# Teque5/caf_cookoff

Measured on NVIDIA B200. Metric: CAF cells/s (400x8192 fp64 surface + peak), higher is better.
Workload: dtype f64

## Files before the change

### caf_cookoff_b200/csrc/caf_kernels.cuh

```cuda
#pragma once
#include <cstdint>
#include <type_traits>
#include "fft16.cuh"

namespace caf {

constexpr int kThreads = 512;
constexpr int kL0 = 4096;
constexpr int kM = 8192;

enum Mode : int {
    kSurface = 0,
    kSpectrumHalf = 1,
    kSpectrumFull = 2,
    kXcorFull = 3,
    kXcorHalf = 4
};

struct PeakOut {
    double value;
    double freq_hz;
    unsigned long long doppler_idx;
    unsigned long long delay_idx;
};

template <typename T>
struct RowArgs {
    const cx<T>* in;
    const cx<T>* in2;
    cx<T>* hperm;
    const double* freqs;
    void* out;
    T* row_peak_val;
    unsigned long long* row_peak_idx;
    PeakOut* peak;
    unsigned long long* peak_words;
    unsigned long long row_offset;
    unsigned int* peak_seq;
    unsigned int seq_val;
    unsigned int* done_counter;
    unsigned int done_last;
    const cx<T>* tw1;
    const cx<T>* tw2;
    const cx<T>* g;
    double dt;
    int L;
    int D;
    int P;
    cx<T>* hshare;
    unsigned int* hflag;
    unsigned int epoch;
    int hprod1;
    const uint4* pull_src;
    uint4* pull_dst;
    unsigned int pull_n16;
    unsigned int* pull_counter;
    unsigned int pull_target;
    unsigned int flags;
    long long* trace;
};

template <typename T> struct Fab;
template <> struct Fab<double> {
    using E = double;
    static constexpr int kRegion = 280;
    static constexpr int kPlane = 16 * kRegion;
    static constexpr int kPipe = 2 * kPlane;
    static __device__ __forceinline__ void st(E* p, int i, double2 v) { p[i] = v.x; p[kPlane + i] = v.y; }
    static __device__ __forceinline__ double2 ld(const E* p, int i) { return make_double2(p[i], p[kPlane + i]); }
};
template <> struct Fab<float> {
    using E = float2;
    static constexpr int kRegion = 256;
    static constexpr int kPipe = 16 * kRegion;
    static __device__ __forceinline__ void st(E* p, int i, float2 v) { p[i] = v; }
    static __device__ __forceinline__ float2 ld(const E* p, int i) { return p[i]; }
};

template <typename T>
struct SmemLayout {
    static constexpr size_t kS = sizeof(typename Fab<T>::E) * 2 * Fab<T>::kPipe;
    static constexpr size_t kPtab = sizeof(cx<T>) * 2 * 2 * 48;
    static constexpr size_t kRed = 16 * 8 + 16 * 8;
    static constexpr size_t kCand = 2 * 256 * (8 + 4);
    static constexpr size_t kMisc = 64;
    static constexpr size_t kNeedle = sizeof(T) * 2 * kL0;
    static constexpr size_t offPtab = kS, offRed = offPtab + kPtab, offCand = offRed + kRed, offMisc = offCand + kCand,
                            offNeedle = offMisc + kMisc;
    static constexpr size_t kTotalNoNeedle = offNeedle;
    static constexpr size_t kTotal = offNeedle + kNeedle;
};

template <typename T>
struct Ctx {
    static constexpr bool kPadded = std::is_same<T, double>::value;
    typename Fab<T>::E* Sr;
    cx<T>* ptab;
    uint32_t tm_A;
    uint32_t tm_B;
    uint32_t tm_g;
    int w, lane, r, h, t;
    int wb;
    int hs[2];
    int hr;
    long long* tr;

    __device__ __forceinline__ void init(unsigned char* smem_raw, int tid) {
        const int hw_warp = tid >> 5;
        lane = tid & 31; r = tid >> 8;
        h = (lane & 7) | ((lane >> 1) & 8);
        const int sub = (lane >> 3) & 1;
        w = 2 * (hw_warp & 7) + sub;
        t = 16 * w + h;
        wb = Fab<T>::kRegion * w;
        hs[0] = h ^ (sub << 3); hs[1] = hs[0] ^ 8;
        hr = h ^ (((sub ^ h) & 1) << 3);
        Sr = reinterpret_cast<typename Fab<T>::E*>(smem_raw) + r * Fab<T>::kPipe;
        ptab = nullptr; tm_A = tm_B = tm_g = 0; tr = nullptr;
    }
    __device__ __forceinline__ int ix_block(int k) const {
        if constexpr (kPadded) return k * Fab<T>::kRegion + (t ^ ((t & 16) >> 1));
        else return k * 256 + 16 * w + hs[k & 1];
    }
    __device__ __forceinline__ int ix_own(int i) const {
        if constexpr (kPadded) return wb + 16 * i + (h ^ ((i & 1) << 3));
        else return wb + 16 * i + hs[i & 1];
    }
    __device__ __forceinline__ int ix_tw(int k) const {
        if constexpr (kPadded) return wb + 17 * k + h;
        else return wb + 16 * k + (hs[k & 1] ^ k);
    }
    __device__ __forceinline__ int ix_tr(int m) const {
        if constexpr (kPadded) return wb + 17 * h + m;
        else return wb + 16 * h + (m ^ hr);
    }
};

#ifdef CAF_TRACE
#define CAF_TR(c_, slot_) do { if ((c_).tr && (c_).lane == 0) (c_).tr[slot_] = clock64(); } while (0)
#else
#define CAF_TR(c_, slot_) do { } while (0)
#endif

__device__ __forceinline__ void tmem_ld_x16(uint32_t taddr, uint32_t (&r)[16]) {
    asm volatile("tcgen05.ld.sync.aligned.32x32b.x16.b32 {%0,%1,%2,%3,%4,%5,%6,%7,%8,%9,%10,%11,%12,%13,%14,%15}, [%16];\n"
                 : "=r"(r[0]), "=r"(r[1]), "=r"(r[2]), "=r"(r[3]), "=r"(r[4]), "=r"(r[5]), "=r"(r[6]), "=r"(r[7]),
                   "=r"(r[8]), "=r"(r[9]), "=r"(r[10]), "=r"(r[11]), "=r"(r[12]), "=r"(r[13]), "=r"(r[14]), "=r"(r[15])
                 : "r"(taddr) : "memory");
}
__device__ __forceinline__ void tmem_st_x16(uint32_t taddr, const uint32_t (&r)[16]) {
    asm volatile("tcgen05.st.sync.aligned.32x32b.x16.b32 [%0], {%1,%2,%3,%4,%5,%6,%7,%8,%9,%10,%11,%12,%13,%14,%15,%16};\n"
                 :: "r"(taddr), "r"(r[0]), "r"(r[1]), "r"(r[2]), "r"(r[3]), "r"(r[4]), "r"(r[5]), "r"(r[6]), "r"(r[7]),
                    "r"(r[8]), "r"(r[9]), "r"(r[10]), "r"(r[11]), "r"(r[12]), "r"(r[13]), "r"(r[14]), "r"(r[15]) : "memory");
}
__device__ __forceinline__ void tmem_ld_x8(uint32_t taddr, uint32_t (&r)[8]) {
    asm volatile("tcgen05.ld.sync.aligned.32x32b.x8.b32 {%0,%1,%2,%3,%4,%5,%6,%7}, [%8];\n"
                 : "=r"(r[0]), "=r"(r[1]), "=r"(r[2]), "=r"(r[3]), "=r"(r[4]), "=r"(r[5]), "=r"(r[6]), "=r"(r[7])
                 : "r"(taddr) : "memory");
}
__device__ __forceinline__ void tmem_st_x8(uint32_t taddr, const uint32_t (&r)[8]) {
    asm volatile("tcgen05.st.sync.aligned.32x32b.x8.b32 [%0], {%1,%2,%3,%4,%5,%6,%7,%8};\n"
                 :: "r"(taddr), "r"(r[0]), "r"(r[1]), "r"(r[2]), "r"(r[3]), "r"(r[4]), "r"(r[5]), "r"(r[6]), "r"(r[7]) : "memory");
}
__device__ __forceinline__ void tmem_wait_ld() { asm volatile("tcgen05.wait::ld.sync.aligned;\n" ::: "memory"); }
__device__ __forceinline__ void tmem_wait_st() { asm volatile("tcgen05.wait::st.sync.aligned;\n" ::: "memory"); }

__device__ __forceinline__ void tmem_ld_x4(uint32_t taddr, uint32_t (&r)[4]) {
    asm volatile("tcgen05.ld.sync.aligned.32x32b.x4.b32 {%0,%1,%2,%3}, [%4];\n"
                 : "=r"(r[0]), "=r"(r[1]), "=r"(r[2]), "=r"(r[3]) : "r"(taddr) : "memory");
}
__device__ __forceinline__ void tmem_st_x4(uint32_t taddr, const uint32_t (&r)[4]) {
    asm volatile("tcgen05.st.sync.aligned.32x32b.x4.b32 [%0], {%1,%2,%3,%4};\n"
                 :: "r"(taddr), "r"(r[0]), "r"(r[1]), "r"(r[2]), "r"(r[3]) : "memory");
}
__device__ __forceinline__ void tmem_ld_x2(uint32_t taddr, uint32_t (&r)[2]) {
    asm volatile("tcgen05.ld.sync.aligned.32x32b.x2.b32 {%0,%1}, [%2];\n" : "=r"(r[0]), "=r"(r[1]) : "r"(taddr) : "memory");
}
__device__ __forceinline__ void tmem_st_x2(uint32_t taddr, const uint32_t (&r)[2]) {
    asm volatile("tcgen05.st.sync.aligned.32x32b.x2.b32 [%0], {%1,%2};\n" :: "r"(taddr), "r"(r[0]), "r"(r[1]) : "memory");
}

template <typename T> struct TmemGeom;
template <> struct TmemGeom<double> { static constexpr int kColsPerC = 4, kAlloc = 512; };
template <> struct TmemGeom<float>  { static constexpr int kColsPerC = 2, kAlloc = 256; };

struct Raw4d { uint32_t r[16]; };
struct Raw4f { uint32_t r[8]; };
template <typename T> struct raw4_of;
template <> struct raw4_of<double> { using type = Raw4d; };
template <> struct raw4_of<float>  { using type = Raw4f; };
__device__ __forceinline__ void tmem_ld4_issue(uint32_t taddr, Raw4d& q) { tmem_ld_x16(taddr, q.r); }
__device__ __forceinline__ void tmem_ld4_issue(uint32_t taddr, Raw4f& q) { tmem_ld_x8(taddr, q.r); }
__device__ __forceinline__ void tmem_unpack4(const Raw4d& q, double2 (&o)[4]) {
#pragma unroll
    for (int i = 0; i < 4; ++i) {
        o[i].x = __hiloint2double((int)q.r[4 * i + 1], (int)q.r[4 * i]);
        o[i].y = __hiloint2double((int)q.r[4 * i + 3], (int)q.r[4 * i + 2]);
    }
}
__device__ __forceinline__ void tmem_unpack4(const Raw4f& q, float2 (&o)[4]) {
#pragma unroll
    for (int i = 0; i < 4; ++i) { o[i].x = __uint_as_float(q.r[2 * i]); o[i].y = __uint_as_float(q.r[2 * i + 1]); }
}
__device__ __forceinline__ void tmem_st4(uint32_t taddr, const double2 (&v)[4]) {
    uint32_t r[16];
#pragma unroll
    for (int i = 0; i < 4; ++i) {
        r[4 * i] = (uint32_t)__double2loint(v[i].x); r[4 * i + 1] = (uint32_t)__double2hiint(v[i].x);
        r[4 * i + 2] = (uint32_t)__double2loint(v[i].y); r[4 * i + 3] = (uint32_t)__double2hiint(v[i].y);
    }
    tmem_st_x16(taddr, r);
}
__device__ __forceinline__ void tmem_st4(uint32_t taddr, const float2 (&v)[4]) {
    uint32_t r[8];
#pragma unroll
    for (int i = 0; i < 4; ++i) { r[2 * i] = __float_as_uint(v[i].x); r[2 * i + 1] = __float_as_uint(v[i].y); }
    tmem_st_x8(taddr, r);
}

__device__ __forceinline__ double2 tmem_ld1(uint32_t taddr, double) {
    uint32_t r[4];
    tmem_ld_x4(taddr, r);
    tmem_wait_ld();
    return make_double2(__hiloint2double((int)r[1], (int)r[0]), __hiloint2double((int)r[3], (int)r[2]));
}
__device__ __forceinline__ float2 tmem_ld1(uint32_t taddr, float) {
    uint32_t r[2];
    tmem_ld_x2(taddr, r);
    tmem_wait_ld();
    return make_float2(__uint_as_float(r[0]), __uint_as_float(r[1]));
}
__device__ __forceinline__ void tmem_st1(uint32_t taddr, double2 v) {
    uint32_t r[4] = {(uint32_t)__double2loint(v.x), (uint32_t)__double2hiint(v.x), (uint32_t)__double2loint(v.y), (uint32_t)__double2hiint(v.y)};
    tmem_st_x4(taddr, r);
}
__device__ __forceinline__ void tmem_st1(uint32_t taddr, float2 v) {
    uint32_t r[2] = {__float_as_uint(v.x), __float_as_uint(v.y)};
    tmem_st_x2(taddr, r);
}

template <typename T>
__device__ __forceinline__ cx<T> ldg(const cx<T>* p) { return __ldg(p); }

__device__ __forceinline__ double2 unit_phasor(double n, double phi, double exact_sub) {
    double hi = n * phi;
    double lo = fma(n, phi, -hi);
    double fr = (hi - rint(hi)) + lo - exact_sub;
    fr -= rint(fr);
    double s, c;
    sincospi(2.0 * fr, &s, &c);
    return make_double2(c, s);
}

__device__ __forceinline__ void bar_group(int r) { asm volatile("bar.sync %0, 256;\n" :: "r"(r + 1) : "memory"); }

__device__ __forceinline__ void mbar_init(uint64_t* mb, int count) {
    asm volatile("mbarrier.init.shared::cta.b64 [%0], %1;\n" :: "r"((uint32_t)__cvta_generic_to_shared(mb)), "r"(count) : "memory");
}
__device__ __forceinline__ void mbar_arrive(uint64_t* mb) {
    asm volatile("{\n.reg .b64 st;\nmbarrier.arrive.shared::cta.b64 st, [%0];\n}\n"
                 :: "r"((uint32_t)__cvta_generic_to_shared(mb)) : "memory");
}
__device__ __forceinline__ void mbar_wait(uint64_t* mb, int parity) {
    const uint32_t addr = (uint32_t)__cvta_generic_to_shared(mb);
    asm volatile("{\n.reg .pred p;\nWAIT_%=:\nmbarrier.try_wait.parity.shared::cta.b64 p, [%0], %1;\n@p bra DONE_%=;\nbra WAIT_%=;\nDONE_%=:\n}\n"
                 :: "r"(addr), "r"(parity) : "memory");
}

template <typename T>
__device__ __forceinline__ void tmem_store_power_table(uint32_t taddr, cx<T> w) {
    constexpr int kC = TmemGeom<T>::kColsPerC;
    const cx<T> w2 = csq(w), w4 = csq(w2);
    cx<T> q[4];
    q[0] = mk<T>((T)1, (T)0); q[1] = w4; q[2] = csq(w4); q[3] = cmul(q[2], w4);
    tmem_st4(taddr, q);
    q[0] = w; q[1] = cmul(q[0], w4); q[2] = cmul(q[1], w4); q[3] = cmul(q[2], w4);
    tmem_st4(taddr + 4 * kC, q);
    q[0] = w2; q[1] = cmul(q[0], w4); q[2] = cmul(q[1], w4); q[3] = cmul(q[2], w4);
    tmem_st4(taddr + 8 * kC, q);
    q[0] = cmul(w2, w); q[1] = cmul(q[0], w4); q[2] = cmul(q[1], w4); q[3] = cmul(q[2], w4);
    tmem_st4(taddr + 12 * kC, q);
}

template <typename T, bool INV, int MODE, bool Q0_ONE>
__device__ __forceinline__ void fft16_in_tmem(cx<T> (&v)[16], uint32_t taddr) {
    constexpr int kC = TmemGeom<T>::kColsPerC;
    typename raw4_of<T>::type r0, r1, r2, r3;
    cx<T> q[4];
    tmem_ld4_issue(taddr, r0);
    tmem_wait_ld();
    tmem_ld4_issue(taddr + 4 * kC, r1);
    tmem_unpack4(r0, q);
    radix4_in<T, INV, MODE, Q0_ONE>(v[0], v[4], v[8], v[12], q[0], q[1], q[2], q[3]);
    tmem_wait_ld();
    tmem_ld4_issue(taddr + 8 * kC, r2);
    tmem_unpack4(r1, q);
    radix4_in<T, INV, MODE, false>(v[1], v[5], v[9], v[13], q[0], q[1], q[2], q[3]);
    tmem_wait_ld();
    tmem_ld4_issue(taddr + 12 * kC, r3);
    tmem_unpack4(r2, q);
    radix4_in<T, INV, MODE, false>(v[2], v[6], v[10], v[14], q[0], q[1], q[2], q[3]);
    tmem_wait_ld();
    tmem_unpack4(r3, q);
    radix4_in<T, INV, MODE, false>(v[3], v[7], v[11], v[15], q[0], q[1], q[2], q[3]);
    fft16_stage_b<T, INV>(v);
}

template <typename T, int MODE>
__device__ __forceinline__ void mul_table_tmem(cx<T> (&v)[16], uint32_t taddr) {
    constexpr int kC = TmemGeom<T>::kColsPerC;
    typename raw4_of<T>::type r0, r1, r2, r3;
    cx<T> q[4];
    tmem_ld4_issue(taddr, r0);
    tmem_ld4_issue(taddr + 4 * kC, r1);
    tmem_wait_ld();
    tmem_ld4_issue(taddr + 8 * kC, r2);
    tmem_ld4_issue(taddr + 12 * kC, r3);
    tmem_unpack4(r0, q);
#pragma unroll
    for (int a = 1; a < 4; ++a) v[4 * a] = tw_apply<MODE>(v[4 * a], q[a]);
    tmem_unpack4(r1, q);
#pragma unroll
    for (int a = 0; a < 4; ++a) v[1 + 4 * a] = tw_apply<MODE>(v[1 + 4 * a], q[a]);
    tmem_wait_ld();
    tmem_unpack4(r2, q);
#pragma unroll
    for (int a = 0; a < 4; ++a) v[2 + 4 * a] = tw_apply<MODE>(v[2 + 4 * a], q[a]);
    tmem_unpack4(r3, q);
#pragma unroll
    for (int a = 0; a < 4; ++a) v[3 + 4 * a] = tw_apply<MODE>(v[3 + 4 * a], q[a]);
}

template <typename T, typename Hook, typename Hook3>
__device__ __forceinline__ void forward_tail(cx<T> (&v)[16], const Ctx<T>& c,
                                             uint64_t* empty_mb, int empty_parity, Hook&& hook, Hook3&& hook3) {
    mul_table_tmem<T, kTwMul>(v, c.tm_A);
    CAF_TR(c, 3);
    if (empty_mb) mbar_wait(empty_mb, empty_parity);
    hook();
    bar_group(c.r);
#pragma unroll
    for (int k = 0; k < 16; ++k) Fab<T>::st(c.Sr, c.ix_block(k), v[k]);
    CAF_TR(c, 4);
    bar_group(c.r);
#pragma unroll
    for (int i = 0; i < 16; ++i) v[i] = Fab<T>::ld(c.Sr, c.ix_own(i));
    CAF_TR(c, 5);

    fft16<T, false>(v);
    CAF_TR(c, 6);
    __syncwarp();
#pragma unroll
    for (int k = 0; k < 16; ++k) Fab<T>::st(c.Sr, c.ix_tw(k), v[k]);
    __syncwarp();
#pragma unroll
    for (int m = 0; m < 16; ++m) v[m] = Fab<T>::ld(c.Sr, c.ix_tr(m));
    hook3();
    CAF_TR(c, 7);

    fft16_in_tmem<T, false, kTwMul, true>(v, c.tm_B);
    CAF_TR(c, 8);
}
template <typename T, typename Hook, typename Hook3>
__device__ __forceinline__ void forward_4096(cx<T> (&v)[16], const Ctx<T>& c,
                                             uint64_t* empty_mb, int empty_parity, Hook&& hook, Hook3&& hook3) {
    fft16<T, false>(v);
    forward_tail<T>(v, c, empty_mb, empty_parity, hook, hook3);
}

template <typename T, bool HFUSED>
__device__ __forceinline__ void inverse_4096(cx<T> (&v)[16], const Ctx<T>& c, uint32_t tm_h) {
    if constexpr (HFUSED) fft16_in_tmem<T, true, kTwConjX, false>(v, tm_h);
    else fft16<T, true>(v);
    CAF_TR(c, 10);
    __syncwarp();
#pragma unroll
    for (int k = 0; k < 16; ++k) Fab<T>::st(c.Sr, c.ix_tw(k), v[k]);
    __syncwarp();
#pragma unroll
    for (int m = 0; m < 16; ++m) v[m] = Fab<T>::ld(c.Sr, c.ix_tr(m));
    CAF_TR(c, 11);

    fft16_in_tmem<T, true, kTwMulConj, true>(v, c.tm_B);
    CAF_TR(c, 12);
    __syncwarp();
#pragma unroll
    for (int k = 0; k < 16; ++k) Fab<T>::st(c.Sr, c.ix_own(k), v[k]);
    CAF_TR(c, 13);
    bar_group(c.r);
#pragma unroll
    for (int k = 0; k < 16; ++k) v[k] = Fab<T>::ld(c.Sr, c.ix_block(k));
    CAF_TR(c, 14);

    fft16_in_tmem<T, true, kTwMulConj, true>(v, c.tm_A);
    CAF_TR(c, 15);
}

template <typename T, int J>
__device__ __forceinline__ cx<T> mul_w32_inv(cx<T> a) {
    constexpr T Cc[8] = {(T)1.0L, (T)0.98078528040323044913L, (T)0.92387953251128675613L, (T)0.83146961230254523708L,
                         (T)0.70710678118654752440L, (T)0.55557023301960222474L, (T)0.38268343236508977173L,
                         (T)0.19509032201612826785L};
    constexpr T Ss[8] = {(T)0.0L, (T)0.19509032201612826785L, (T)0.38268343236508977173L, (T)0.55557023301960222474L,
                         (T)0.70710678118654752440L, (T)0.83146961230254523708L, (T)0.92387953251128675613L,
                         (T)0.98078528040323044913L};
    if constexpr (J == 0) return a;
    else if constexpr (J == 8) return mk<T>(-a.y, a.x);
    else if constexpr (J < 8) return mk<T>(a.x * Cc[J] - a.y * Ss[J], a.x * Ss[J] + a.y * Cc[J]);
    else return mk<T>(-a.x * Ss[J - 8] - a.y * Cc[J - 8], a.x * Cc[J - 8] - a.y * Ss[J - 8]);
}

__device__ __forceinline__ void pack_peak_words(const PeakOut& p, unsigned long long global_row_offset,
                                                unsigned long long* __restrict__ words) {
    words[0] = (unsigned long long)__double_as_longlong(p.value);
    words[1] = (p.doppler_idx == ~0ull) ? ~0ull : p.doppler_idx + global_row_offset;
    words[2] = p.delay_idx;
    words[3] = (unsigned long long)__double_as_longlong(p.freq_hz);
}

template <typename T>
__device__ __forceinline__ void amax_take(T& best, int& bidx, T m, int k) {
    if (m > best || (m == best && k < bidx)) { best = m; bidx = k; }
}

template <int I> using ic = std::integral_constant<int, I>;

template <typename T, int MODE, bool FULL, bool SHARED = false>
__global__ void __launch_bounds__(kThreads, 1) caf_rows_kernel(const RowArgs<T> a) {
    using C = cx<T>;
    using SL = SmemLayout<T>;
    using TG = TmemGeom<T>;
    extern __shared__ __align__(16) unsigned char smem_raw[];
    C* ptab = reinterpret_cast<C*>(smem_raw + SL::offPtab);
    unsigned long long* red_idx = reinterpret_cast<unsigned long long*>(smem_raw + SL::offRed);
    double* red_val = reinterpret_cast<double*>(smem_raw + SL::offRed + 128);
    double* cand_val = reinterpret_cast<double*>(smem_raw + SL::offCand);
    int* cand_idx = reinterpret_cast<int*>(smem_raw + SL::offCand + 2 * 256 * 8);
    uint32_t* misc = reinterpret_cast<uint32_t*>(smem_raw + SL::offMisc);
    uint64_t* mb_full = reinterpret_cast<uint64_t*>(smem_raw + SL::offMisc + 16);
    uint64_t* mb_empty = reinterpret_cast<uint64_t*>(smem_raw + SL::offMisc + 24);

    const int tid = threadIdx.x;
#ifdef CAF_TRACE
    long long tr_g0 = 0, tr_c0 = clock64();
    asm volatile("mov.u64 %0, %%globaltimer;" : "=l"(tr_g0));
#endif
    Ctx<T> c;
    const int hw_warp = tid >> 5;
    c.init(smem_raw, tid);
    c.ptab = ptab;
    const int w = c.w, lane = c.lane, r = c.r, h = c.h, t = c.t, tg = tid & 255, wg = hw_warp & 7;

    constexpr bool kHalfZero = (MODE == kSurface || MODE == kSpectrumHalf || MODE == kXcorHalf);
    constexpr bool kWritesH = (MODE == kSpectrumHalf || MODE == kSpectrumFull);
    constexpr bool kUseTmem = (MODE == kSurface);
    T* const ndl_re = reinterpret_cast<T*>(smem_raw + SL::offNeedle);
    T* const ndl_im = ndl_re + kL0;

    const int rows_per_pair = (MODE == kSurface) ? a.D : 1;
    const long long n_items = (long long)a.P * rows_per_pair;
    const int lo = (int)(n_items * blockIdx.x / gridDim.x), hi = (int)(n_items * (blockIdx.x + 1) / gridDim.x);
    int pair = lo / rows_per_pair, row = lo - pair * rows_per_pair;

    int buf = 0;
    int cur_pair = -1;
    int posts = 0;
    bool drain_pending = false;
    bool h_from_share = false;
    C v[16];

    if constexpr (MODE == kSurface) asm volatile("griddepcontrol.launch_dependents;\n" ::: "memory");
    const C tb0 = ldg<T>(a.tw1 + 256 + t), tb1 = ldg<T>(a.tw2 + 16 + h), tb4 = ldg<T>(a.g + t);
    bool preloaded = false;
    double phi_first = 0.0;
    if constexpr (MODE == kSurface) {
        if (lo < hi) {
            const bool producer0 = !SHARED || (int)blockIdx.x == ((r == 0) ? 0 : a.hprod1);
            const C* src = (producer0 ? a.in2 : a.in) + (long long)pair * a.L;
#pragma unroll
            for (int q = 0; q < (int)sizeof(C) / 8; ++q) {
                const long long byte0 = ((long long)tg + 256 * q) * 128;
                if (byte0 < (long long)a.L * (long long)sizeof(C))
                    asm volatile("prefetch.global.L2 [%0];\n" :: "l"(reinterpret_cast<const char*>(src) + byte0));
            }
            if (tg == 255) asm volatile("prefetch.global.L2 [%0];\n" :: "l"(a.freqs + row));
        }
    }

    uint4 pulled = make_uint4(0u, 0u, 0u, 0u);
    const unsigned int pull_i = blockIdx.x * 64u + (unsigned int)(tid - 448);
    if constexpr (MODE == kSurface && SHARED) {
        if (a.pull_src != nullptr && tid >= 448 && pull_i < a.pull_n16)
            asm volatile("ld.volatile.global.v4.u32 {%0,%1,%2,%3}, [%4];\n"
                         : "=r"(pulled.x), "=r"(pulled.y), "=r"(pulled.z), "=r"(pulled.w) : "l"(a.pull_src + pull_i) : "memory");
    }

    if (tid == 0) {
        mbar_init(mb_full, 256);
        mbar_init(mb_empty, 256);
        asm volatile("fence.mbarrier_init.release.cluster;\n" ::: "memory");
    }

    uint32_t tm_h = 0;
    {
        if (hw_warp == 0) {
            asm volatile("tcgen05.alloc.cta_group::1.sync.aligned.shared::cta.b32 [%0], %1;\n"
                         :: "l"((uint64_t)__cvta_generic_to_shared(&misc[0])), "n"(TG::kAlloc));
            asm volatile("tcgen05.relinquish_alloc_permit.cta_group::1.sync.aligned;\n");
        }
        asm volatile("tcgen05.fence::before_thread_sync;\n");
        __syncthreads();
        asm volatile("tcgen05.fence::after_thread_sync;\n");
        const uint32_t base = misc[0] + ((uint32_t)(32 * (hw_warp & 3)) << 16);
        const int j = hw_warp >> 2;
        tm_h = base + (uint32_t)((16 * j) * TG::kColsPerC);
        c.tm_A = base + (uint32_t)((64 + 16 * (j & 1)) * TG::kColsPerC);
        c.tm_B = base + (uint32_t)(96 * TG::kColsPerC);
        c.tm_g = base + (uint32_t)((112 + 4 * j) * TG::kColsPerC);
        if (r == 0) tmem_store_power_table<T>(c.tm_A, tb0);
        else if (j == 2) tmem_store_power_table<T>(c.tm_B, tb1);
        tmem_st1(c.tm_g, tb4);
        tmem_wait_st();
        asm volatile("tcgen05.fence::before_thread_sync;\n");
        __syncthreads();
        asm volatile("tcgen05.fence::after_thread_sync;\n");
    }

    if constexpr (MODE == kSurface) {
        if (!(SHARED && (a.flags & 1u))) asm volatile("griddepcontrol.wait;\n" ::: "memory");
        if constexpr (SHARED) {
            if (a.pull_src != nullptr) {
                if (tid >= 448) {
                    unsigned int i = pull_i;
                    if (i < a.pull_n16) __stcg(a.pull_dst + i, pulled);
                    for (i += gridDim.x * 64u; i < a.pull_n16; i += gridDim.x * 64u) {
                        uint4 q;
                        asm volatile("ld.volatile.global.v4.u32 {%0,%1,%2,%3}, [%4];\n"
                                     : "=r"(q.x), "=r"(q.y), "=r"(q.z), "=r"(q.w) : "l"(a.pull_src + i) : "memory");
                        __stcg(a.pull_dst + i, q);
                    }
                    __threadfence();
                    __syncwarp();
                    if (lane == 0) asm volatile("red.release.gpu.global.add.u32 [%0], 1;\n" :: "l"(a.pull_counter) : "memory");
                }
                if (tid == 0) {
                    unsigned int seen;
                    do {
                        asm volatile("ld.acquire.gpu.global.u32 %0, [%1];\n" : "=r"(seen) : "l"(a.pull_counter) : "memory");
                    } while ((int)(seen - a.pull_target) < 0);
                }
                __syncthreads();
            }
        }
        if (lo < hi) {
            const bool producer0 = !SHARED || (int)blockIdx.x == ((r == 0) ? 0 : a.hprod1);
            const C* src = (producer0 ? a.in2 : a.in) + (long long)pair * a.L;
#pragma unroll
            for (int i = 0; i < 16; ++i) {
                const int n = t + 256 * i;
                v[i] = (n < a.L) ? (SHARED ? __ldcg(src + n) : ldg<T>(src + n)) : mk<T>((T)0, (T)0);
            }
            preloaded = true;
            phi_first = (SHARED ? __ldcg(a.freqs + row) : __ldg(a.freqs + row)) * a.dt;
        }
    }

    auto fill_ptab = [&](int buf, double phi) {
        if (tg < 48) {
            const int e = tg, which = e >> 4, idx = e & 15;
            const int n = idx << (which == 0 ? 8 : which == 1 ? 4 : 0);
            double2 p = unit_phasor((double)n, phi, (double)(r * n) * (1.0 / 8192.0));
            ptab[(buf * 2 + r) * 48 + e] = mk<T>((T)p.x, (T)p.y);
        }
    };
    auto fill_ptab_both = [&](int buf, double phi) {
        if (tg < 96) {
            const int rr = tg >= 48, e = tg - 48 * rr, which = e >> 4, idx = e & 15;
            const int n = idx << (which == 0 ? 8 : which == 1 ? 4 : 0);
            double2 p = unit_phasor((double)n, phi, (double)(rr * n) * (1.0 / 8192.0));
            ptab[(buf * 2 + rr) * 48 + e] = mk<T>((T)p.x, (T)p.y);
        }
    };
    auto phasor_fft16 = [&](C (&v)[16], int buf) {
        const C* pt = ptab + (buf * 2 + r) * 48;
        const C s4 = pt[4];
        const C base = cmul(pt[16 + w], pt[32 + h]);
        {
            const C q1 = cmul(base, s4), q2 = cmul(q1, s4), q3 = cmul(q2, s4);
            radix4_in<T, false, kTwMul, false>(v[0], v[4], v[8], v[12], base, q1, q2, q3);
        }
#pragma unroll
        for (int cc = 1; cc < 4; ++cc) {
            const C q0 = cmul(base, pt[cc]), q1 = cmul(q0, s4), q2 = cmul(q1, s4), q3 = cmul(q2, s4);
            radix4_in<T, false, kTwMul, false>(v[cc], v[cc + 4], v[cc + 8], v[cc + 12], q0, q1, q2, q3);
        }
        fft16_stage_b<T, false>(v);
    };
    auto load_half = [&](C (&v)[16], const C* src, int L) {
#pragma unroll
        for (int i = 0; i < 16; ++i) {
            const int n = t + 256 * i;
            v[i] = (n < L) ? ldg<T>(src + n) : mk<T>((T)0, (T)0);
        }
    };


    auto fold_candidates = [&](int slot, int it) {
        double bv = 0.0;
        int bi = 0x7fffffff;
#pragma unroll
        for (int q = 0; q < 8; ++q) {
            const double cv = cand_val[slot * 256 + lane + 32 * q];
            const int ci = cand_idx[slot * 256 + lane + 32 * q];
            amax_take<double>(bv, bi, cv, ci);
        }
#pragma unroll
        for (int off = 16; off > 0; off >>= 1) {
            double ov = __shfl_xor_sync(0xffffffffu, bv, off);
            int oi = __shfl_xor_sync(0xffffffffu, bi, off);
            amax_take<double>(bv, bi, ov, oi);
        }
        if (lane == 0) {
            if (!(bv > 0.0)) bi = 0;
            if (a.row_peak_val) a.row_peak_val[it] = (T)bv;
            if (a.row_peak_idx) a.row_peak_idx[it] = (unsigned long long)bi;
        }
    };

    auto empty_gate = [&](uint64_t*& mb, int& par) {
        if (r == 1 && drain_pending) { mb = mb_empty; par = (posts - 1) & 1; drain_pending = false; }
        else { mb = nullptr; par = 0; }
    };

    c.tr = nullptr;
    for (int item = lo; item < hi; ++item, buf ^= 1) {
#ifdef CAF_TRACE
        c.tr = (a.trace && item - lo < 8) ? a.trace + ((((long long)blockIdx.x * 16 + hw_warp) * 8 + (item - lo)) * 32) : nullptr;
#endif
        CAF_TR(c, 0);
        if constexpr (MODE == kSurface) {
            if (pair != cur_pair) {
                cur_pair = pair;
                constexpr bool shared_h = SHARED;
                const int my_prod_cta = (r == 0) ? 0 : a.hprod1;
                const bool producer = !shared_h || (int)blockIdx.x == my_prod_cta;
                const bool park = shared_h && a.hprod1 != 0 && ((int)blockIdx.x == 0 || (int)blockIdx.x == a.hprod1);
                bar_group(r);
                if (producer) {
                    fill_ptab(buf, 0.0);
                    if (!preloaded) load_half(v, a.in2 + (long long)pair * a.L, a.L);
                    preloaded = false;
                }
                bar_group(r);
                if (producer) {
#ifdef CAF_TRACE
                    long long* tr_row = c.tr;
                    if (a.trace && item == lo) c.tr = a.trace + ((((long long)blockIdx.x * 16 + hw_warp) * 8 + 7) * 32);
#endif
                    CAF_TR(c, 0);
                    phasor_fft16(v, buf);
                    uint64_t* mb; int par;
                    empty_gate(mb, par);
                    forward_tail<T>(v, c, mb, par, [&] {
                                        if (r == 1 && mb != nullptr && wg == 3) fold_candidates((buf ^ 1) & 1, item - 1);
                                    }, []{});
                    const T sc = (T)(1.0 / 8192.0);
#pragma unroll
                    for (int q = 0; q < 4; ++q) {
                        C tmp[4];
#pragma unroll
                        for (int i = 0; i < 4; ++i) {
                            tmp[i] = mk<T>(v[q + 4 * i].x * sc, v[q + 4 * i].y * sc);
                            if (shared_h) __stcg(a.hshare + (q + 4 * i) * kThreads + tid, tmp[i]);
                        }
                        tmem_st4(tm_h + 4 * q * TG::kColsPerC, tmp);
                    }
                    if (shared_h) {
                        __threadfence();
                        bar_group(r);
                        if (tg == 0) asm volatile("st.release.gpu.global.u32 [%0], %1;\n" :: "l"(a.hflag + r), "r"(a.epoch) : "memory");
                    }
                    CAF_TR(c, 9);
#ifdef CAF_TRACE
                    c.tr = tr_row;
#endif
                } else {
                    h_from_share = true;
                }
                if (park) __syncthreads();
                if (!preloaded) load_half(v, a.in + (long long)pair * a.L, a.L);
                const bool first_row_phi = preloaded || (item == lo);
                preloaded = false;
                __syncthreads();
                {
                    T* const dst = (r == 0) ? ndl_re : ndl_im;
#pragma unroll
                    for (int i = 0; i < 16; ++i) dst[t + 256 * i] = (r == 0) ? v[i].x : v[i].y;
                }
                fill_ptab(buf, first_row_phi ? phi_first : a.freqs[row] * a.dt);
                __syncthreads();
            }
            CAF_TR(c, 1);
#pragma unroll
            for (int i = 0; i < 16; ++i) v[i] = mk<T>(ndl_re[t + 256 * i], ndl_im[t + 256 * i]);
            phasor_fft16(v, buf);
            CAF_TR(c, 2);
        } else if constexpr (kHalfZero) {
            bar_group(r);
            fill_ptab(buf, 0.0);
            load_half(v, a.in + (long long)pair * a.L, a.L);
            bar_group(r);
            phasor_fft16(v, buf);
        } else {
            const C* src = a.in + (long long)pair * kM;
#pragma unroll
            for (int i = 0; i < 16; ++i) {
                const int n = t + 256 * i;
                C x0 = ldg<T>(src + n), x1 = ldg<T>(src + n + kL0);
                if (r == 0) v[i] = cadd(x0, x1);
                else v[i] = cmulc(csub(x0, x1), ldg<T>(a.g + n));
            }
            fft16<T, false>(v);
        }

        {
            uint64_t* mb; int par;
            empty_gate(mb, par);
            const bool had_mail = (mb != nullptr);
            forward_tail<T>(v, c, mb, par, [&] {
                                    if constexpr (MODE == kSurface) {
                                        if (r == 1) {
                                            if ((item + 1 < hi) && (row + 1 < a.D)) fill_ptab_both(buf ^ 1, a.freqs[row + 1] * a.dt);
                                            if (had_mail && wg == 3) fold_candidates((buf ^ 1) & 1, item - 1);
                                        }
                                    }
                                },
                                [&] {
                                    if constexpr (kUseTmem) {
                                        if (SHARED && h_from_share && lane == 0) {
                                            unsigned int seen;
                                            do {
                                                asm volatile("ld.acquire.gpu.global.u32 %0, [%1];\n" : "=r"(seen) : "l"(a.hflag + r) : "memory");
                                            } while ((int)(seen - a.epoch) < 0);
                                        }
                                    }
                                });
        }

        C* hp = a.hperm + (long long)pair * kM;
        if constexpr (kWritesH) {
            const T sc = (T)(1.0 / 8192.0);
#pragma unroll
            for (int k = 0; k < 16; ++k) hp[((k * 16 + w) * 2 + r) * 16 + h] = mk<T>(v[k].x * sc, v[k].y * sc);
        } else {
            if constexpr (kUseTmem) {
                if (SHARED && h_from_share) {
                    h_from_share = false;
                    __syncwarp();
#pragma unroll
                    for (int k = 0; k < 16; ++k) Fab<T>::st(c.Sr, c.ix_own(k), v[k]);
#pragma unroll
                    for (int k = 0; k < 16; ++k) v[k] = __ldcg(a.hshare + k * kThreads + tid);
#pragma unroll
                    for (int q = 0; q < 4; ++q) {
                        C hv[4];
#pragma unroll
                        for (int i = 0; i < 4; ++i) hv[i] = v[q + 4 * i];
                        tmem_st4(tm_h + 4 * q * TG::kColsPerC, hv);
                    }
#pragma unroll
                    for (int k = 0; k < 16; ++k) v[k] = Fab<T>::ld(c.Sr, c.ix_own(k));
                    tmem_wait_st();
                }
                CAF_TR(c, 9);
                inverse_4096<T, true>(v, c, tm_h);
            } else {
#pragma unroll
                for (int k = 0; k < 16; ++k) v[k] = cmulc(ldg<T>(hp + ((k * 16 + w) * 2 + r) * 16 + h), v[k]);
                CAF_TR(c, 9);
                inverse_4096<T, false>(v, c, 0u);
            }

            if (r == 1) {
                const C gt = tmem_ld1(c.tm_g, T());
                auto post = [&](auto jt) {
                    constexpr int j = decltype(jt)::value;
                    v[j] = cmul(v[j], mul_w32_inv<T, j>(gt));
                };
                post(ic<0>{}); post(ic<1>{}); post(ic<2>{}); post(ic<3>{}); post(ic<4>{}); post(ic<5>{}); post(ic<6>{}); post(ic<7>{});
                post(ic<8>{}); post(ic<9>{}); post(ic<10>{}); post(ic<11>{}); post(ic<12>{}); post(ic<13>{}); post(ic<14>{}); post(ic<15>{});
                CAF_TR(c, 16);
                bar_group(1);
#pragma unroll
                for (int k = 0; k < 16; ++k) Fab<T>::st(c.Sr, c.ix_block(k), v[k]);
                mbar_arrive(mb_full);
                CAF_TR(c, 17);
                ++posts;
                drain_pending = true;

            } else {
                const int L = FULL ? kL0 : a.L;
                const int nout = 2 * L, skip = kM - nout;
                T* orow = (MODE == kSurface && a.out) ? reinterpret_cast<T*>(a.out) + item * (long long)nout : nullptr;
                C* ocx = (MODE != kSurface) ? reinterpret_cast<C*>(a.out) + (long long)pair * kM : nullptr;
                T best0 = (T)0, best1 = (T)0;
                int bidx0 = 0, bidx1 = 0;
                auto emit = [&](C y, int kp, T& best, int& bidx) {
                    if constexpr (MODE == kSurface) {
                        const T m = y.x * y.x + y.y * y.y;
                        if constexpr (FULL) {
                            if (orow) orow[kp] = m;
                            if (m > best) { best = m; bidx = kp; }
                        } else {
                            int k = -1;
                            if (kp <= L) k = kp; else if (kp > kM - L) k = kp - skip;
                            if (k >= 0 && k < nout) {
                                if (orow) orow[k] = m;
                                if (m > best) { best = m; bidx = k; }
                            }
                        }
                    } else {
                        ocx[kp] = y;
                    }
                };
                CAF_TR(c, 16);
                mbar_wait(mb_full, posts & 1);
                CAF_TR(c, 17);
                const typename Fab<T>::E* mail = c.Sr + Fab<T>::kPipe;
#pragma unroll
                for (int k = 0; k < 16; ++k) {
                    const C Bp = Fab<T>::ld(mail, c.ix_block(k));
                    const int n = t + 256 * k;
                    emit(cadd(v[k], Bp), n, best0, bidx0);
                    emit(csub(v[k], Bp), n + kL0, best1, bidx1);
                }
                if constexpr (MODE == kSurface) {
                    T best = best0;
                    int bidx = bidx0;
                    if (best1 > best) { best = best1; bidx = bidx1; }
                    cand_val[(buf & 1) * 256 + tg] = (double)best;
                    cand_idx[(buf & 1) * 256 + tg] = bidx;
                }
                mbar_arrive(mb_empty);
                CAF_TR(c, 18);
                ++posts;
            }
        }
        CAF_TR(c, 19);
        if (++row == rows_per_pair) { row = 0; ++pair; }
    }
    if constexpr (MODE == kSurface) {
        if (r == 1 && drain_pending) {
            mbar_wait(mb_empty, (posts - 1) & 1);
            if (wg == 3) fold_candidates((buf ^ 1) & 1, hi - 1);
        }
    }

    {
        asm volatile("tcgen05.fence::before_thread_sync;\n");
        __syncthreads();
        if (hw_warp == 0) {
            asm volatile("tcgen05.dealloc.cta_group::1.sync.aligned.b32 %0, %1;\n" :: "r"(misc[0]), "n"(TG::kAlloc));
        }
    }

#ifdef CAF_TRACE
    if (a.trace && (tid & 31) == 0) {
        long long g1; asm volatile("mov.u64 %0, %%globaltimer;" : "=l"(g1));
        long long* q = a.trace + (((long long)blockIdx.x * 16 + hw_warp) * 8 + 0) * 32;
        q[20] = tr_g0; q[21] = g1; q[22] = tr_c0; q[23] = clock64();
    }
#endif
    if constexpr (MODE == kSurface) {
        if (SHARED && a.peak != nullptr && a.done_counter != nullptr && r == 1 && wg == 3) {
            unsigned int last = 0;
            if (lane == 0) {
                __threadfence();
                last = (atomicAdd(a.done_counter, 1u) == a.done_last) ? 1u : 0u;
            }
            last = __shfl_sync(0xffffffffu, last, 0);
            if (last) {
                __threadfence();
                double best = 0.0;
                int brow = 0x7fffffff;
                for (int d0 = 0; d0 < a.D; d0 += 128) {
                    double vv[4];
#pragma unroll
                    for (int q = 0; q < 4; ++q) {
                        const int d = d0 + 32 * q + lane;
                        vv[q] = (d < a.D) ? (double)__ldcg(a.row_peak_val + d) : 0.0;
                    }
#pragma unroll
                    for (int q = 0; q < 4; ++q)
                        if (vv[q] > best) { best = vv[q]; brow = d0 + 32 * q + lane; }
                }
#pragma unroll
                for (int off = 16; off > 0; off >>= 1) {
                    double ov = __shfl_xor_sync(0xffffffffu, best, off);
                    int oi = __shfl_xor_sync(0xffffffffu, brow, off);
                    amax_take<double>(best, brow, ov, oi);
                }
                if (lane == 0) {
                    PeakOut p;
                    if (best > 0.0 && brow != 0x7fffffff) {
                        p.value = best; p.freq_hz = a.freqs[brow];
                        p.doppler_idx = (unsigned long long)brow; p.delay_idx = __ldcg(a.row_peak_idx + brow);
                    } else {
                        p.value = 0.0; p.freq_hz = 0.0; p.doppler_idx = ~0ull; p.delay_idx = 0;
                    }
                    *a.peak = p;
                    if (a.peak_words) pack_peak_words(p, a.row_offset, a.peak_words);
                    if (a.peak_seq) {
                        __threadfence_system();
                        *reinterpret_cast<volatile unsigned int*>(a.peak_seq) = a.seq_val;
                    }
                }
            }
        }
    }
#ifdef CAF_TRACE
    if (a.trace && tid == 0) {
        long long g2; asm volatile("mov.u64 %0, %%globaltimer;" : "=l"(g2));
        a.trace[(((long long)blockIdx.x * 16 + 0) * 8 + 0) * 32 + 29] = g2;
    }
#endif
}

template <typename T>
__global__ void __launch_bounds__(256) caf_peak_kernel(const T* __restrict__ row_val,
                                                       const unsigned long long* __restrict__ row_idx,
                                                       const double* __restrict__ freqs, int D, PeakOut* out,
                                                       unsigned long long* words = nullptr,
                                                       unsigned long long row_offset = 0ull) {
    __shared__ double sv[8];
    __shared__ int si[8];
    const long long base = (long long)blockIdx.x * D;
    double best = 0.0;
    int brow = 0x7fffffff;
    for (int d = threadIdx.x; d < D; d += blockDim.x) {
        double v = (double)row_val[base + d];
        if (v > best) { best = v; brow = d; }
    }
#pragma unroll
    for (int off = 16; off > 0; off >>= 1) {
        double ov = __shfl_xor_sync(0xffffffffu, best, off);
        int oi = __shfl_xor_sync(0xffffffffu, brow, off);
        amax_take<double>(best, brow, ov, oi);
    }
    if ((threadIdx.x & 31) == 0) { sv[threadIdx.x >> 5] = best; si[threadIdx.x >> 5] = brow; }
    __syncthreads();
    if (threadIdx.x == 0) {
        for (int q = 1; q < 8; ++q) amax_take<double>(best, brow, sv[q], si[q]);
        PeakOut p;
        if (best > 0.0 && brow != 0x7fffffff) {
            p.value = best; p.freq_hz = freqs[brow];
            p.doppler_idx = (unsigned long long)brow; p.delay_idx = row_idx[base + brow];
        } else {
            p.value = 0.0; p.freq_hz = 0.0; p.doppler_idx = ~0ull; p.delay_idx = 0;
        }
        if (out) out[blockIdx.x] = p;
        if (words && blockIdx.x == 0) pack_peak_words(p, row_offset, words);
    }
}

__global__ void caf_peak_pack_kernel(const PeakOut* __restrict__ local, unsigned long long global_row_offset,
                                     unsigned long long* __restrict__ words) {
    if (threadIdx.x == 0) {
        PeakOut p;
        if (local) p = *local;
        else { p.value = 0.0; p.freq_hz = 0.0; p.doppler_idx = ~0ull; p.delay_idx = 0; }
        pack_peak_words(p, global_row_offset, words);
    }
}

constexpr unsigned long long kPeakNone = ~0ull, kPeakRemoteError = ~0ull - 1ull;
__global__ void caf_peak_resolve_kernel(const unsigned long long* __restrict__ words, int world, PeakOut* out,
                                        int* __restrict__ status) {
    if (threadIdx.x != 0) return;
    PeakOut best; best.value = 0.0; best.freq_hz = 0.0; best.doppler_idx = ~0ull; best.delay_idx = 0;
    int st = 0;
    for (int r = 0; r < world; ++r) {
        const unsigned long long* w = words + 4 * r;
        if (w[1] == kPeakRemoteError) { st = 1; continue; }
        if (w[1] == kPeakNone) continue;
        const double v = __longlong_as_double((long long)w[0]);
        if (v > best.value || (v == best.value && v > 0.0 && w[1] < best.doppler_idx)) {
            best.value = v; best.freq_hz = __longlong_as_double((long long)w[3]); best.doppler_idx = w[1]; best.delay_idx = w[2];
        }
    }
    *out = best;
    if (status) *status = st;
}

__global__ void caf_peak_exchange_kernel(const unsigned long long* __restrict__ send, unsigned long long* const* __restrict__ peer_mail,
                                         unsigned long long* mail, int world, int rank, unsigned long long epoch,
                                         PeakOut* out, int* __restrict__ status) {
    const int lane = threadIdx.x;
    const size_t par = (size_t)(epoch & 1ull);
    const unsigned long long w0 = send[0], w1 = send[1], w2 = send[2], w3 = send[3];
    for (int s = lane; s < world; s += 32) {
        unsigned long long* dst = peer_mail[s] + (par * world + rank) * 8;
        asm volatile("st.volatile.global.v2.u64 [%0], {%1, %2};\n" :: "l"(dst), "l"(w0), "l"(w1) : "memory");
        asm volatile("st.volatile.global.v2.u64 [%0], {%1, %2};\n" :: "l"(dst + 2), "l"(w2), "l"(w3) : "memory");
        __threadfence_system();
        asm volatile("st.release.sys.global.u64 [%0], %1;\n" :: "l"(dst + 4), "l"(epoch) : "memory");
    }
    double bv = 0.0, bf = 0.0;
    unsigned long long brow = ~0ull, bdel = 0ull;
    int st = 0;
    for (int s = lane; s < world; s += 32) {
        const unsigned long long* src = mail + (par * world + s) * 8;
        unsigned long long tag = 0ull;
        unsigned int polls = 0;
        for (;;) {
            asm volatile("ld.acquire.sys.global.u64 %0, [%1];\n" : "=l"(tag) : "l"(src + 4) : "memory");
            if (tag == epoch) break;
            if (++polls == (1u << 27)) { st = 1; break; }
        }
        if (tag != epoch) continue;
        unsigned long long r0, r1, r2, r3;
        asm volatile("ld.volatile.global.v2.u64 {%0, %1}, [%2];\n" : "=l"(r0), "=l"(r1) : "l"(src) : "memory");
        asm volatile("ld.volatile.global.v2.u64 {%0, %1}, [%2];\n" : "=l"(r2), "=l"(r3) : "l"(src + 2) : "memory");
        if (r1 == kPeakRemoteError) { st = 1; continue; }
        if (r1 == kPeakNone) continue;
        const double v = __longlong_as_double((long long)r0);
        if (v > bv || (v == bv && v > 0.0 && r1 < brow)) { bv = v; bf = __longlong_as_double((long long)r3); brow = r1; bdel = r2; }
    }
#pragma unroll
    for (int off = 16; off > 0; off >>= 1) {
        const double ov = __shfl_xor_sync(0xffffffffu, bv, off), of = __shfl_xor_sync(0xffffffffu, bf, off);
        const unsigned long long orow = __shfl_xor_sync(0xffffffffu, brow, off), odel = __shfl_xor_sync(0xffffffffu, bdel, off);
        st |= __shfl_xor_sync(0xffffffffu, st, off);
        if (ov > bv || (ov == bv && ov > 0.0 && orow < brow)) { bv = ov; bf = of; brow = orow; bdel = odel; }
    }
    if (lane == 0) {
        PeakOut best; best.value = bv; best.freq_hz = bf; best.doppler_idx = brow; best.delay_idx = bdel;
        *out = best;
        if (status) *status = st;
    }
}

template <typename T>
__global__ void __launch_bounds__(256) caf_layout_kernel(const T* __restrict__ rust, T* __restrict__ out, int L, int W,
                                                         int lag0, T* __restrict__ row_val,
                                                         unsigned long long* __restrict__ row_idx) {
    __shared__ double sv[8];
    __shared__ int si[8];
    const long long row = blockIdx.x;
    const T* src = rust + row * 2LL * L;
    T* dst = out + row * (long long)W;
    double best = 0.0;
    int bidx = 0x7fffffff;
    for (int j = threadIdx.x; j < W; j += blockDim.x) {
        int k = lag0 - j;
        if (k < 0) k += 2 * L;
        const T m = sqrt(src[k]);
        dst[j] = m;
        if ((double)m > best) { best = (double)m; bidx = j; }
    }
#pragma unroll
    for (int off = 16; off > 0; off >>= 1) {
        double ov = __shfl_xor_sync(0xffffffffu, best, off);
        int oi = __shfl_xor_sync(0xffffffffu, bidx, off);
        amax_take<double>(best, bidx, ov, oi);
    }
    if ((threadIdx.x & 31) == 0) { sv[threadIdx.x >> 5] = best; si[threadIdx.x >> 5] = bidx; }
    __syncthreads();
    if (threadIdx.x == 0) {
        for (int q = 1; q < 8; ++q) amax_take<double>(best, bidx, sv[q], si[q]);
        if (!(best > 0.0)) bidx = 0;
        row_val[row] = (T)best;
        row_idx[row] = (unsigned long long)bidx;
    }
}

template <typename T>
__global__ void caf_apply_shift_kernel(const cx<T>* __restrict__ in, cx<T>* __restrict__ out, long long n,
                                       double phi ) {
    for (long long i = blockIdx.x * (long long)blockDim.x + threadIdx.x; i < n;
         i += (long long)gridDim.x * blockDim.x) {
        double2 p = unit_phasor((double)i, phi, 0.0);
        cx<T> x = in[i];
        out[i] = mk<T>((T)((double)x.x * p.x - (double)x.y * p.y), (T)((double)x.x * p.y + (double)x.y * p.x));
    }
}

__global__ void caf_widen_c64_kernel(const float2* __restrict__ in, double2* __restrict__ out, long long n) {
    for (long long i = blockIdx.x * (long long)blockDim.x + threadIdx.x; i < n; i += (long long)gridDim.x * blockDim.x) {
        const float2 x = in[i];
        out[i] = make_double2((double)x.x, (double)x.y);
    }
}

template <typename T>
__global__ void caf_fold_circular_kernel(const cx<T>* __restrict__ y, cx<T>* __restrict__ out, int n, int big_n) {
    int k = blockIdx.x * blockDim.x + threadIdx.x;
    if (k < n) {
        cx<T> a = y[k];
        cx<T> b = (k == 0) ? mk<T>((T)0, (T)0) : y[big_n - n + k];
        out[k] = cadd(a, b);
    }
}

template <typename T>
__global__ void __launch_bounds__(512) caf_fma_probe_kernel(T* sink, int iters, T seed) {
    T a0 = seed + (T)threadIdx.x, a1 = a0 + (T)1, a2 = a0 + (T)2, a3 = a0 + (T)3;
    T a4 = a0 + (T)4, a5 = a0 + (T)5, a6 = a0 + (T)6, a7 = a0 + (T)7;
    const T m = (T)0.999999, c = (T)1e-6;
    for (int i = 0; i < iters; ++i) {
#pragma unroll
        for (int u = 0; u < 8; ++u) {
            a0 = fma(a0, m, c); a1 = fma(a1, m, c); a2 = fma(a2, m, c); a3 = fma(a3, m, c);
            a4 = fma(a4, m, c); a5 = fma(a5, m, c); a6 = fma(a6, m, c); a7 = fma(a7, m, c);
        }
    }
    T r = ((a0 + a1) + (a2 + a3)) + ((a4 + a5) + (a6 + a7));
    if (r == (T)123456789) sink[0] = r;
}

}
```

Before: 96.16 billion.

## Split final radix-2 combine across both warpgroups with paired mbarriers

Before, one warpgroup posted its whole half-spectrum to shared memory and the other did all the final butterfly, magnitude, store and argmax work. Now each warpgroup publishes half of its outputs, waits on the peer's mailbox through a per-group mbarrier, and computes half of the output cells. Candidate buffers are duplicated and the fold reduces over both. This balances the epilogue between the two groups but adds mbarrier pairs, extra shared memory, and a cross-group handshake that is sensitive to parity tracking.

```diff
diff --git a/caf_cookoff_b200/csrc/caf_kernels.cuh b/caf_cookoff_b200/csrc/caf_kernels.cuh
--- a/caf_cookoff_b200/csrc/caf_kernels.cuh
+++ b/caf_cookoff_b200/csrc/caf_kernels.cuh
@@ -88,7 +88,8 @@
     static constexpr size_t offPtab = kS, offRed = offPtab + kPtab, offCand = offRed + kRed, offMisc = offCand + kCand,
                             offNeedle = offMisc + kMisc;
     static constexpr size_t kTotalNoNeedle = offNeedle;
-    static constexpr size_t kTotal = offNeedle + kNeedle;
+    static constexpr size_t offCand1 = offNeedle + kNeedle;
+    static constexpr size_t kTotal = offCand1 + kCand;
 };
 
 template <typename T>
@@ -337,7 +338,9 @@
     mul_table_tmem<T, kTwMul>(v, c.tm_A);
     CAF_TR(c, 3);
     if (empty_mb) mbar_wait(empty_mb, empty_parity);
+    CAF_TR(c, 24);
     hook();
+    CAF_TR(c, 25);
     bar_group(c.r);
 #pragma unroll
     for (int k = 0; k < 16; ++k) Fab<T>::st(c.Sr, c.ix_block(k), v[k]);
@@ -434,11 +437,9 @@
     C* ptab = reinterpret_cast<C*>(smem_raw + SL::offPtab);
     unsigned long long* red_idx = reinterpret_cast<unsigned long long*>(smem_raw + SL::offRed);
     double* red_val = reinterpret_cast<double*>(smem_raw + SL::offRed + 128);
-    double* cand_val = reinterpret_cast<double*>(smem_raw + SL::offCand);
-    int* cand_idx = reinterpret_cast<int*>(smem_raw + SL::offCand + 2 * 256 * 8);
     uint32_t* misc = reinterpret_cast<uint32_t*>(smem_raw + SL::offMisc);
     uint64_t* mb_full = reinterpret_cast<uint64_t*>(smem_raw + SL::offMisc + 16);
-    uint64_t* mb_empty = reinterpret_cast<uint64_t*>(smem_raw + SL::offMisc + 24);
+    uint64_t* mb_empty = reinterpret_cast<uint64_t*>(smem_raw + SL::offMisc + 32);
 
     const int tid = threadIdx.x;
 #ifdef CAF_TRACE
@@ -464,7 +465,6 @@
 
     int buf = 0;
     int cur_pair = -1;
-    int posts = 0;
     bool drain_pending = false;
     bool h_from_share = false;
     C v[16];
@@ -497,7 +497,9 @@
 
     if (tid == 0) {
         mbar_init(mb_full, 256);
+        mbar_init(mb_full + 1, 256);
         mbar_init(mb_empty, 256);
+        mbar_init(mb_empty + 1, 256);
         asm volatile("fence.mbarrier_init.release.cluster;\n" ::: "memory");
     }
 
@@ -605,14 +607,20 @@
     };
 
 
+    auto cand_val = [&](int g) { return reinterpret_cast<double*>(smem_raw + (g ? SL::offCand1 : SL::offCand)); };
+    auto cand_idx = [&](int g) { return reinterpret_cast<int*>(smem_raw + (g ? SL::offCand1 : SL::offCand) + 2 * 256 * 8); };
     auto fold_candidates = [&](int slot, int it) {
+        mbar_wait(mb_empty, buf ^ 1);
         double bv = 0.0;
         int bi = 0x7fffffff;
-#pragma unroll
-        for (int q = 0; q < 8; ++q) {
-            const double cv = cand_val[slot * 256 + lane + 32 * q];
-            const int ci = cand_idx[slot * 256 + lane + 32 * q];
-            amax_take<double>(bv, bi, cv, ci);
+#pragma unroll 1
+        for (int g = 0; g < 2; ++g) {
+#pragma unroll
+            for (int q = 0; q < 8; ++q) {
+                const double cv = cand_val(g)[slot * 256 + lane + 32 * q];
+                const int ci = cand_idx(g)[slot * 256 + lane + 32 * q];
+                amax_take<double>(bv, bi, cv, ci);
+            }
         }
 #pragma unroll
         for (int off = 16; off > 0; off >>= 1) {
@@ -628,7 +636,7 @@
     };
 
     auto empty_gate = [&](uint64_t*& mb, int& par) {
-        if (r == 1 && drain_pending) { mb = mb_empty; par = (posts - 1) & 1; drain_pending = false; }
+        if (drain_pending) { mb = mb_empty + r; par = buf ^ 1; drain_pending = false; }
         else { mb = nullptr; par = 0; }
     };
 
@@ -736,6 +744,7 @@
                                     }
                                 },
                                 [&] {
+
                                     if constexpr (kUseTmem) {
                                         if (SHARED && h_from_share && lane == 0) {
                                             unsigned int seen;
@@ -781,77 +790,75 @@
                 inverse_4096<T, false>(v, c, 0u);
             }
 
-            if (r == 1) {
+            const int L = FULL ? kL0 : a.L;
+            const int nout = 2 * L, skip = kM - nout;
+            T* orow = (MODE == kSurface && a.out) ? reinterpret_cast<T*>(a.out) + item * (long long)nout : nullptr;
+            C* ocx = (MODE != kSurface) ? reinterpret_cast<C*>(a.out) + (long long)pair * kM : nullptr;
+            T best0 = (T)0, best1 = (T)0;
+            int bidx0 = 0, bidx1 = 0;
+            auto emit = [&](C y, int kp, T& best, int& bidx) {
+                if constexpr (MODE == kSurface) {
+                    const T m = y.x * y.x + y.y * y.y;
+                    if constexpr (FULL) {
+                        if (orow) orow[kp] = m;
+                        if (m > best) { best = m; bidx = kp; }
+                    } else {
+                        int k = -1;
+                        if (kp <= L) k = kp; else if (kp > kM - L) k = kp - skip;
+                        if (k >= 0 && k < nout) {
+                            if (orow) orow[k] = m;
+                            if (m > best) { best = m; bidx = k; }
+                        }
+                    }
+                } else {
+                    ocx[kp] = y;
+                }
+            };
+            const typename Fab<T>::E* mail = c.Sr + (r ? -Fab<T>::kPipe : Fab<T>::kPipe);
+            auto radix2 = [&](auto k0c) {
+                constexpr int K0 = decltype(k0c)::value, KP = 8 - K0;
+#pragma unroll
+                for (int j = 0; j < 8; ++j) Fab<T>::st(c.Sr, c.ix_block(KP + j), v[KP + j]);
+                mbar_arrive(mb_full + r);
+                CAF_TR(c, 16);
                 const C gt = tmem_ld1(c.tm_g, T());
-                auto post = [&](auto jt) {
-                    constexpr int j = decltype(jt)::value;
-                    v[j] = cmul(v[j], mul_w32_inv<T, j>(gt));
+                auto tw = [&](auto jt) { constexpr int k = decltype(jt)::value; v[k] = cmul(v[k], mul_w32_inv<T, k>(gt)); };
+                if constexpr (K0 == 8) {
+                    tw(ic<8>{}); tw(ic<9>{}); tw(ic<10>{}); tw(ic<11>{}); tw(ic<12>{}); tw(ic<13>{}); tw(ic<14>{}); tw(ic<15>{});
+                }
+                mbar_wait(mb_full + (r ^ 1), buf);
+                CAF_TR(c, 17);
+                auto cell = [&](auto jt) {
+                    constexpr int k = K0 + decltype(jt)::value;
+                    const C o = Fab<T>::ld(mail, c.ix_block(k));
+                    C A, Bp;
+                    if constexpr (K0 == 8) { A = o; Bp = v[k]; }
+                    else { A = v[k]; Bp = cmul(o, mul_w32_inv<T, k>(gt)); }
+                    const int n = t + 256 * k;
+                    emit(cadd(A, Bp), n, best0, bidx0);
+                    emit(csub(A, Bp), n + kL0, best1, bidx1);
                 };
-                post(ic<0>{}); post(ic<1>{}); post(ic<2>{}); post(ic<3>{}); post(ic<4>{}); post(ic<5>{}); post(ic<6>{}); post(ic<7>{});
-                post(ic<8>{}); post(ic<9>{}); post(ic<10>{}); post(ic<11>{}); post(ic<12>{}); post(ic<13>{}); post(ic<14>{}); post(ic<15>{});
-                CAF_TR(c, 16);
-                bar_group(1);
-#pragma unroll
-                for (int k = 0; k < 16; ++k) Fab<T>::st(c.Sr, c.ix_block(k), v[k]);
-                mbar_arrive(mb_full);
-                CAF_TR(c, 17);
-                ++posts;
-                drain_pending = true;
-
-            } else {
-                const int L = FULL ? kL0 : a.L;
-                const int nout = 2 * L, skip = kM - nout;
-                T* orow = (MODE == kSurface && a.out) ? reinterpret_cast<T*>(a.out) + item * (long long)nout : nullptr;
-                C* ocx = (MODE != kSurface) ? reinterpret_cast<C*>(a.out) + (long long)pair * kM : nullptr;
-                T best0 = (T)0, best1 = (T)0;
-                int bidx0 = 0, bidx1 = 0;
-                auto emit = [&](C y, int kp, T& best, int& bidx) {
-                    if constexpr (MODE == kSurface) {
-                        const T m = y.x * y.x + y.y * y.y;
-                        if constexpr (FULL) {
-                            if (orow) orow[kp] = m;
-                            if (m > best) { best = m; bidx = kp; }
-                        } else {
-                            int k = -1;
-                            if (kp <= L) k = kp; else if (kp > kM - L) k = kp - skip;
-                            if (k >= 0 && k < nout) {
-                                if (orow) orow[k] = m;
-                                if (m > best) { best = m; bidx = k; }
-                            }
-                        }
-                    } else {
-                        ocx[kp] = y;
-                    }
-                };
-                CAF_TR(c, 16);
-                mbar_wait(mb_full, posts & 1);
-                CAF_TR(c, 17);
-                const typename Fab<T>::E* mail = c.Sr + Fab<T>::kPipe;
-#pragma unroll
-                for (int k = 0; k < 16; ++k) {
-                    const C Bp = Fab<T>::ld(mail, c.ix_block(k));
-                    const int n = t + 256 * k;
-                    emit(cadd(v[k], Bp), n, best0, bidx0);
-                    emit(csub(v[k], Bp), n + kL0, best1, bidx1);
-                }
-                if constexpr (MODE == kSurface) {
-                    T best = best0;
-                    int bidx = bidx0;
-                    if (best1 > best) { best = best1; bidx = bidx1; }
-                    cand_val[(buf & 1) * 256 + tg] = (double)best;
-                    cand_idx[(buf & 1) * 256 + tg] = bidx;
-                }
-                mbar_arrive(mb_empty);
-                CAF_TR(c, 18);
-                ++posts;
+                cell(ic<0>{}); cell(ic<1>{}); cell(ic<2>{}); cell(ic<3>{}); cell(ic<4>{}); cell(ic<5>{}); cell(ic<6>{}); cell(ic<7>{});
+            };
+            if (r == 0) radix2(ic<0>{});
+            else radix2(ic<8>{});
+            if constexpr (MODE == kSurface) {
+                T best = best0;
+                int bidx = bidx0;
+                if (best1 > best) { best = best1; bidx = bidx1; }
+                cand_val(r)[(buf & 1) * 256 + tg] = (double)best;
+                cand_idx(r)[(buf & 1) * 256 + tg] = bidx;
             }
+            mbar_arrive(mb_empty + (r ^ 1));
+            CAF_TR(c, 18);
+            drain_pending = true;
         }
         CAF_TR(c, 19);
         if (++row == rows_per_pair) { row = 0; ++pair; }
     }
     if constexpr (MODE == kSurface) {
         if (r == 1 && drain_pending) {
-            mbar_wait(mb_empty, (posts - 1) & 1);
+            mbar_wait(mb_empty + 1, buf ^ 1);
             if (wg == 3) fold_candidates((buf ^ 1) & 1, hi - 1);
         }
     }
```

Measured after the change: 91.59 billion (median of 6 runs). 0.952x the previous value.
